# diffqc/dqc

Measured on AMD Instinct MI355X. Metric: SCF iterations/sec (Fock build + XC grid) per GPU, cc-pVDZ 20-atom, higher is better.
Workload: dtype f64

## Files before the change

dqc_amd/csrc/grid_density.hip:

```cpp
#include "grid_common.hpp"

namespace dqc {

constexpr int DEN_BM = 64;
constexpr int DEN_NT = DEN_BM * 4;
constexpr int DEN_KC = 16;
constexpr int DEN_SA = DEN_KC + 2;

#ifdef DEN_TRACE
__device__ long long g_den_trace[4 * 16384];
DQC_DEV void den_trace(int k) {
    if (threadIdx.x == 0 && blockIdx.x < 16384) {
        if (k == 0) {
            unsigned hw, xcc;
            asm volatile("s_getreg_b32 %0, hwreg(HW_REG_HW_ID)" : "=s"(hw));
            asm volatile("s_getreg_b32 %0, hwreg(HW_REG_XCC_ID)" : "=s"(xcc));
            g_den_trace[4 * blockIdx.x + 3] = (long long)(((xcc & 7u) << 8) | ((hw >> 8) & 0xffu));
        }
        g_den_trace[4 * blockIdx.x + k] = wall_clock64();
    }
}
#define DEN_TRACE_POINT(k) den_trace(k)
#else
#define DEN_TRACE_POINT(k)
#endif

#ifdef DEN_EXP_UNPAIRED
constexpr bool DEN_PAIRED = false;
#else
constexpr bool DEN_PAIRED = true;
#endif

constexpr int lr_panel_stride(int nct) {
    return (DEN_PAIRED && nct >= 2) ? nct * 16 + 1 : (((nct * 16) & 31) == 16 ? nct * 16 : nct * 16 + 16);
}

template <int NCT, bool GGA, int Q0 = 0>
DQC_DEV void rowdot_epilogue(const v4d (&acc)[NCT], double (&p)[4][GGA ? 4 : 1], const double *__restrict__ blk0,
                             const double *__restrict__ blkg, size_t cs, const int (&roff)[4], int col0) {
    constexpr int NQ = (GGA ? 4 : 1) - Q0, NB = 4 * NQ;
    if (NB == 0) return;
    constexpr int DP = 2;
    double t[DP][NCT];
    auto issue = [&](int bt, double (&dst)[NCT]) {
        const int r = bt / NQ, q = bt % NQ + Q0;
        const double *base = (q == 0 ? blk0 : blkg + q * cs) + col0;
#pragma unroll
        for (int ct = 0; ct < NCT; ct++) dst[ct] = base[roff[r] + ct * 16];
    };
#pragma unroll
    for (int b0 = 0; b0 < DP - 1 && b0 < NB; b0++) issue(b0, t[b0]);
#pragma unroll
    for (int bt = 0; bt < NB; bt++) {
        if (bt + DP - 1 < NB) issue(bt + DP - 1, t[(bt + DP - 1) % DP]);
        const int r = bt / NQ, q = bt % NQ + Q0;
#pragma unroll
        for (int ct = 0; ct < NCT; ct++) p[r][q] += acc[ct][r] * t[bt % DP][ct];
        __builtin_amdgcn_sched_barrier(0);
    }
}

template <int NCT, bool GGA, int Q0 = 0>
DQC_DEV void rowdot_epilogue_paired(const v4d (&acc)[NCT], double (&p)[4][GGA ? 4 : 1], const double *__restrict__ blk0,
                                    const double *__restrict__ blkg, size_t cs, const int (&roff)[4], int lr, int col0) {
    constexpr int NQ = (GGA ? 4 : 1) - Q0, NB = 4 * NQ, NP = NCT / 2, ODD = NCT & 1, DP = 2;
    if (NB == 0) return;
    double2 t2[DP][NP > 0 ? NP : 1];
    double t1[DP];
    auto issue = [&](int bt, double2 (&d2)[NP > 0 ? NP : 1], double &d1) {
        const int r = bt / NQ, q = bt % NQ + Q0;
        const double *base = (q == 0 ? blk0 : blkg + q * cs) + col0;
#pragma unroll
        for (int m = 0; m < NP; m++) d2[m] = *reinterpret_cast<const double2 *>(base + roff[r] + m * 32);
        if (ODD) d1 = base[(roff[r] - lr) + (NCT - 1) * 16];
    };
    issue(0, t2[0], t1[0]);
#pragma unroll
    for (int bt = 0; bt < NB; bt++) {
        if (bt + 1 < NB) issue(bt + 1, t2[(bt + 1) % DP], t1[(bt + 1) % DP]);
        const int r = bt / NQ, q = bt % NQ + Q0;
#pragma unroll
        for (int m = 0; m < NP; m++) p[r][q] += acc[2 * m][r] * t2[bt % DP][m].x + acc[2 * m + 1][r] * t2[bt % DP][m].y;
        if (ODD) p[r][q] += acc[NCT - 1][r] * t1[bt % DP];
        __builtin_amdgcn_sched_barrier(0);
    }
}

template <int NCT>
DQC_DEV void rowdot_epilogue_paired2(const v4d (&acc)[2][NCT], double (&p)[2][4][4], const double *__restrict__ blkg, size_t cs,
                                     const int (&roff)[4], int lr, int col0) {
    constexpr int NQ = 3, NB = 4 * NQ, NP = NCT / 2, ODD = NCT & 1, DP = 2;
    double2 t2[DP][NP > 0 ? NP : 1];
    double t1[DP];
    auto issue = [&](int bt, double2 (&d2)[NP > 0 ? NP : 1], double &d1) {
        const int r = bt / NQ, q = bt % NQ + 1;
        const double *base = blkg + q * cs + col0;
#pragma unroll
        for (int m = 0; m < NP; m++) d2[m] = *reinterpret_cast<const double2 *>(base + roff[r] + m * 32);
        if (ODD) d1 = base[(roff[r] - lr) + (NCT - 1) * 16];
    };
    issue(0, t2[0], t1[0]);
#pragma unroll
    for (int bt = 0; bt < NB; bt++) {
        if (bt + 1 < NB) issue(bt + 1, t2[(bt + 1) % DP], t1[(bt + 1) % DP]);
        const int r = bt / NQ, q = bt % NQ + 1;
#pragma unroll
        for (int sp = 0; sp < 2; sp++) {
#pragma unroll
            for (int m = 0; m < NP; m++) p[sp][r][q] += acc[sp][2 * m][r] * t2[bt % DP][m].x + acc[sp][2 * m + 1][r] * t2[bt % DP][m].y;
            if (ODD) p[sp][r][q] += acc[sp][NCT - 1][r] * t1[bt % DP];
        }
        __builtin_amdgcn_sched_barrier(0);
    }
}

template <int NCT, bool GGA>
__global__ __launch_bounds__(256, 2) void density_kernel(double *__restrict__ rho, double *__restrict__ grho,
                                                         const double *__restrict__ ao, int ngrid, int ld,
                                                         const double *__restrict__ dm, int ntile,
                                                         const double *__restrict__ aoe, int lda) {
    extern __shared__ __attribute__((aligned(16))) double lds[];
    constexpr int LSB = NCT * 16;
    constexpr int LSBP = lr_panel_stride(NCT);
    constexpr int A_SZ = DEN_BM * DEN_SA, B_SZ = DEN_KC * LSBP;
    constexpr int NB2 = (DEN_KC * LSB / 2 + DEN_NT - 1) / DEN_NT;
    constexpr int NKK = DEN_KC / 4;
    double *sA = lds, *sB = lds + 2 * A_SZ;
    const int tid = threadIdx.x, wave = tid >> 6, lane = tid & 63;
    const int lr = lane & 15, lk = lane >> 4;
    const int g0 = blockIdx.x * DEN_BM;
    const size_t cs = (size_t)ngrid * lda;
    const double *aoblk = ao + (size_t)g0 * lda;
    const double *aoeblk = aoe + (size_t)g0 * lda;
    const int rmax = ngrid - 1 - g0;
    const int arow = tid >> 2, aseg = (tid & 3) * 4;
    const int aoff = min(arow, rmax) * lda + aseg;

    double p[4][GGA ? 4 : 1];
#pragma unroll
    for (int r = 0; r < 4; r++)
#pragma unroll
        for (int q = 0; q < (GGA ? 4 : 1); q++) p[r][q] = 0.0;
    int roff[4];
#pragma unroll
    for (int r = 0; r < 4; r++) roff[r] = min(wave * 16 + lk + 4 * r, rmax) * lda + (DEN_PAIRED ? 2 : 1) * lr;

    DEN_TRACE_POINT(0);
    const int nk = ld / DEN_KC;
    for (int jnew = 0; jnew < ntile; jnew += NCT) {
        const int jc = min(jnew, ntile - NCT);
        v4d acc[NCT];
#pragma unroll
        for (int ct = 0; ct < NCT; ct++) acc[ct] = v4d{0, 0, 0, 0};
        double2 paA0 = make_double2(0.0, 0.0), paA1 = paA0, paB0 = paA0, paB1 = paA0, pbA[NB2], pbB[NB2];
        int boff[NB2];
        bool bzero[NB2];
#pragma unroll
        for (int i = 0; i < NB2; i++) {
            const int e = min((tid + i * DEN_NT) * 2, DEN_KC * LSB - 2);
            const int row = e / LSB, col = e - row * LSB;
            boff[i] = row * ld + jc * 16 + col;
            bzero[i] = jc * 16 + col < jnew * 16;
            pbA[i] = pbB[i] = make_double2(0.0, 0.0);
        }
#define DQC_DEN_PREF(KC, S, PART)                                                                          \
    {                                                                                                      \
        const int kq_ = min((KC), nk - 1);      \
        if ((PART) == 0) {                                                                                 \
            const double *s_ = aoblk + kq_ * DEN_KC + aoff;                                                \
            pa##S##0 = *reinterpret_cast<const double2 *>(s_);                                             \
            pa##S##1 = *reinterpret_cast<const double2 *>(s_ + 2);                                         \
        }                                                                                                  \
        const double *d_ = dm + (size_t)kq_ * DEN_KC * ld;                                                 \
        _Pragma("unroll") for (int i = 0; i < NB2; i++) {                                                  \
            if (i % NKK != (PART)) continue;                                                               \
            pb##S[i] = *reinterpret_cast<const double2 *>(d_ + boff[i]);                                   \
            if (bzero[i]) pb##S[i] = make_double2(0.0, 0.0);                                               \
        }                                                                                                  \
    }
#define DQC_DEN_STAGE(KC, S)                                                                               \
    if ((KC) < nk) {                                                                                       \
        const int buf_ = (KC) & 1;                                                                         \
        double *a_ = sA + buf_ * A_SZ + arow * DEN_SA + aseg;                                              \
        *reinterpret_cast<double2 *>(a_) = pa##S##0;                                                       \
        *reinterpret_cast<double2 *>(a_ + 2) = pa##S##1;                                                   \
        _Pragma("unroll") for (int i = 0; i < NB2; i++) {                                                  \
            const int e = (tid + i * DEN_NT) * 2;                                                          \
            const int row = e / LSB, col = e - row * LSB;                                                  \
            if (row < DEN_KC) {                                     \
                double *d = sB + buf_ * B_SZ + row * LSBP + col;                                           \
                d[0] = pb##S[i].x;                                                                         \
                d[1] = pb##S[i].y;                                                                         \
            }                                                                                              \
        }                                                                                                  \
    }
#define DQC_DEN_MFMAS(KC, S)                                                                               \
    {                                                                                                      \
        const int buf_ = (KC) & 1;                                                                         \
        const double *a = sA + buf_ * A_SZ + (wave * 16 + lr) * DEN_SA + lk;                               \
        const double *b = sB + buf_ * B_SZ + lk * LSBP + lr;                                               \
        const double *b2 = b + lr;  \
        _Pragma("unroll") for (int kk = 0; kk < NKK; kk++) {                                               \
            DQC_DEN_PREF((KC) + 2, S, kk)                     \
            const double av = a[kk * 4];                                                                   \
            _Pragma("unroll") for (int ct = 0; ct < NCT; ct++) {                                           \
                const double bv = (DEN_PAIRED && ct < 2 * (NCT / 2)) ? b2[kk * 4 * LSBP + 32 * (ct >> 1) + (ct & 1)] \
                                                                    : b[kk * 4 * LSBP + ct * 16];          \
                acc[ct] = mfma_f64(av, bv, acc[ct]);                                                       \
            }                                                                                              \
        }                                                                                                  \
    }
        __syncthreads();
#pragma unroll
        for (int part = 0; part < NKK; part++) DQC_DEN_PREF(0, A, part)
#pragma unroll
        for (int part = 0; part < NKK; part++) DQC_DEN_PREF(1, B, part)
        DQC_DEN_STAGE(0, A)
        __syncthreads();
        int kc = 0;
        for (; kc + 1 < nk; kc += 2) {
            DQC_DEN_MFMAS(kc, A)
            DQC_DEN_STAGE(kc + 1, B)
            __syncthreads();
            DQC_DEN_MFMAS(kc + 1, B)
            DQC_DEN_STAGE(kc + 2, A)
            __syncthreads();
        }
        if (kc < nk) {
            DQC_DEN_MFMAS(kc, A)
            __syncthreads();
        }
#undef DQC_DEN_PREF
// ... 187 lines not shown
        rs += __shfl_xor(rs, 32);
        const int row = g0 + wave * 16 + lr;
        if (lk == 0 && row < ngrid) rho[(size_t)sp * ngrid + row] = rs;
    }
    if (!GGA) return;

    double p[NS][4][GGA ? 4 : 1];
#pragma unroll
    for (int sp = 0; sp < NS; sp++)
#pragma unroll
    for (int r = 0; r < 4; r++)
#pragma unroll
        for (int q = 0; q < (GGA ? 4 : 1); q++) p[sp][r][q] = 0.0;
    int roff[4];
#pragma unroll
    for (int r = 0; r < 4; r++) roff[r] = min(wave * 16 + lk + 4 * r, rmax) * lda + (DEN_PAIRED ? 2 : 1) * lr;

    for (int jnew = 0; jnew < ntile; jnew += NCT) {
        const int jc = min(jnew, ntile - NCT);
        v4d acc[NS][NCT];
#pragma unroll
        for (int sp = 0; sp < NS; sp++)
#pragma unroll
        for (int ct = 0; ct < NCT; ct++) acc[sp][ct] = v4d{0, 0, 0, 0};
        double2 pb[NB2];
        int boff[NB2];
        bool bzero[NB2];
#pragma unroll
        for (int i = 0; i < NB2; i++) {
            const int e = min((tid + i * DEN_NT) * 2, DEN_KC * LSB - 2);
            const int row = e / LSB, col = e - row * LSB;
            boff[i] = row * ld + jc * 16 + col;
            bzero[i] = jc * 16 + col < jnew * 16;
        }
        auto prefetch = [&](int kc) {
            const double *l = orbt + (size_t)kc * DEN_KC * ld;
#pragma unroll
            for (int i = 0; i < NB2; i++) {
                pb[i] = *reinterpret_cast<const double2 *>(l + boff[i]);
                if (bzero[i]) pb[i] = make_double2(0.0, 0.0);
            }
        };
        auto stage = [&](int buf) {
#pragma unroll
            for (int i = 0; i < NB2; i++) {
                const int e = (tid + i * DEN_NT) * 2;
                const int row = e / LSB, col = e - row * LSB;
                if (row < DEN_KC) {
                    double *d = sB + buf * B_SZ + row * LSBP + col;
                    d[0] = pb[i].x;
                    d[1] = pb[i].y;
                }
            }
        };
        __syncthreads();
        prefetch(0);
        stage(0);
        __syncthreads();
#pragma unroll 1
        for (int kc = 0; kc < NRT; kc++) {
            const int buf = kc & 1;
            if (kc + 1 < NRT) prefetch(kc + 1);
            v4d a4 = a1[0];
#pragma unroll
            for (int c = 1; c < NRT; c++)
                if (kc == c) a4 = a1[c];
            const double *b = sB + buf * B_SZ + lk * LSBP + lr;
            const double *b2 = b + lr;
#pragma unroll
            for (int kk = 0; kk < 4; kk++) {
                const double av = a4[kk];
#pragma unroll
                for (int ct = 0; ct < NCT; ct++) {
                    const double bv = (DEN_PAIRED && ct < 2 * (NCT / 2)) ? b2[kk * 4 * LSBP + 32 * (ct >> 1) + (ct & 1)]
                                                                        : b[kk * 4 * LSBP + ct * 16];
                    if (NS == 1 || kc < NRU) acc[0][ct] = mfma_f64(av, bv, acc[0][ct]);
                    else acc[NS - 1][ct] = mfma_f64(av, bv, acc[NS - 1][ct]);
                }
            }
            if (kc + 1 < NRT) stage(buf ^ 1);
            __syncthreads();
        }
        DEN_TRACE_POINT(1);
        if constexpr (NS == 2) {
            static_assert(NS == 1 || (DEN_PAIRED && GGA), "spin-fused form: paired epilogue only");
            rowdot_epilogue_paired2<NCT>(acc, p, aoblk, cs, roff, lr, jc * 16);
        } else if constexpr (!DEN_PAIRED) rowdot_epilogue<NCT, GGA, 1>(acc[0], p[0], aoblk, aoblk, cs, roff, jc * 16);
        else if constexpr (GGA) rowdot_epilogue_paired<NCT, true, 1>(acc[0], p[0], aoblk, aoblk, cs, roff, lr, jc * 16);
        DEN_TRACE_POINT(2);
    }
#pragma unroll
    for (int sp = 0; sp < NS; sp++)
#pragma unroll
    for (int r = 0; r < 4; r++)
#pragma unroll
        for (int q = 0; q < (GGA ? 4 : 1); q++) {
            double v = p[sp][r][q];
            v += __shfl_xor(v, 1);
            v += __shfl_xor(v, 2);
            v += __shfl_xor(v, 4);
            v += __shfl_xor(v, 8);
            p[sp][r][q] = v;
        }
    if (lr == 0) {
#pragma unroll
        for (int sp = 0; sp < NS; sp++)
#pragma unroll
        for (int r = 0; r < 4; r++) {
            const int row = g0 + wave * 16 + lk + 4 * r;
            if (row < ngrid) {
                double *gs = grho + (size_t)sp * 3 * ngrid;
                gs[row] = 2.0 * p[sp][r][1];
                gs[(size_t)ngrid + row] = 2.0 * p[sp][r][2];
                gs[2 * (size_t)ngrid + row] = 2.0 * p[sp][r][3];
            }
        }
    }
}

template <int NRT, int NCT>
static constexpr size_t density_lr_lds_bytes() {
    constexpr int LSBP = lr_panel_stride(NCT);
    constexpr int RPS = LrGeom<NRT>::RPS;
    return sizeof(double) * 2 * (DEN_BM * DEN_SA + DEN_KC * (LSBP > RPS ? LSBP : RPS));
}

constexpr int lr_max_nct(int nrt) { return nrt <= 3 ? 14 : (nrt <= 4 ? 12 : 10); }

template <int NRT, bool GGA>
static int launch_density_lr_n(int nct, dim3 grid, hipStream_t st, double *rho, double *grho, const double *ao, int ngrid,
                               int ld, const double *orb, const double *orbt, int ntile, int lda) {
#define DQC_DLR_CASE(N)                                                                                          \
    case N:                                                                                                      \
        if constexpr (!GGA || N <= lr_max_nct(NRT)) {          \
            constexpr size_t shm = density_lr_lds_bytes<NRT, N>();                                               \
            auto kern = density_lr_kernel<NRT, N, GGA>;                                                          \
            (void)hipFuncSetAttribute((const void *)kern, hipFuncAttributeMaxDynamicSharedMemorySize, (int)shm); \
            hipLaunchKernelGGL(kern, grid, dim3(DEN_NT), shm, st, rho, grho, ao, ngrid, ld, orb, orbt, ntile, lda); \
            return 0;                                                                                            \
        }                                                                                                        \
        break;
    switch (nct) {
        DQC_DLR_CASE(1) DQC_DLR_CASE(2) DQC_DLR_CASE(3) DQC_DLR_CASE(4) DQC_DLR_CASE(5) DQC_DLR_CASE(6) DQC_DLR_CASE(7)
        DQC_DLR_CASE(8) DQC_DLR_CASE(9) DQC_DLR_CASE(10) DQC_DLR_CASE(11) DQC_DLR_CASE(12) DQC_DLR_CASE(13) DQC_DLR_CASE(14)
        DQC_DLR_CASE(15) DQC_DLR_CASE(16)
    default:
        break;
    }
#undef DQC_DLR_CASE
    set_error("density_lr: internal tile-count dispatch error");
    return DQC_EINVAL;
}

template <int NRT>
__global__ __launch_bounds__(256, 2) void density_lr_tau_kernel(double *__restrict__ rho, double *__restrict__ grho, double *__restrict__ tau,
                                                                const double *__restrict__ ao, int ngrid, int ld,
                                                                const double *__restrict__ orb, int lda) {
    extern __shared__ __attribute__((aligned(16))) double lds[];
    constexpr int RP = LrGeom<NRT>::RP, RPS = LrGeom<NRT>::RPS;
    constexpr int A_SZ = DEN_BM * DEN_SA, B_SZ = DEN_KC * RPS;
    constexpr int NL2 = (DEN_KC * RP / 2 + DEN_NT - 1) / DEN_NT;
    static_assert(NL2 <= 4, "L chunk wider than 4 double2 per thread");
    double *sA = lds, *sB = lds + 4 * A_SZ;
    const int tid = threadIdx.x, wave = tid >> 6, lane = tid & 63;
    const int lr = lane & 15, lk = lane >> 4;
    const int g0 = blockIdx.x * DEN_BM;
    const size_t cs = (size_t)ngrid * lda;
    const double *aoblk = ao + (size_t)g0 * lda;
    const int rmax = ngrid - 1 - g0;
    const int arow = tid >> 2, aseg = (tid & 3) * 4;
    const int aoff = min(arow, rmax) * lda + aseg;
    const int nk = ld / DEN_KC;
    const int lo0 = min((tid + 0 * DEN_NT) * 2, DEN_KC * RP - 2), lo1 = min((tid + 1 * DEN_NT) * 2, DEN_KC * RP - 2);
    const int lo2 = min((tid + 2 * DEN_NT) * 2, DEN_KC * RP - 2), lo3 = min((tid + 3 * DEN_NT) * 2, DEN_KC * RP - 2);

    v4d psi[NRT];
    double rs = 0.0, ts = 0.0, gs[3] = {0.0, 0.0, 0.0};
#pragma unroll 1
    for (int pair = 0; pair < 2; pair++) {
        const double *blk0 = aoblk + (size_t)(2 * pair) * cs, *blk1 = blk0 + cs;
        v4d a0[NRT], a1[NRT];
#pragma unroll
        for (int ct = 0; ct < NRT; ct++) a0[ct] = a1[ct] = v4d{0, 0, 0, 0};
        double2 x0a, x0b, y0a, y0b, x1a, x1b, y1a, y1b, pl0a, pl0b, pl0c, pl0d, pl1a, pl1b, pl1c, pl1d;
        pl0a = pl0b = pl0c = pl0d = pl1a = pl1b = pl1c = pl1d = make_double2(0.0, 0.0);
#define DQC_LT_PREFETCH(KC, S)                                                                            \
    {                                                                                                     \
        const int kq = min((KC), nk - 1);      \
        const double *s0_ = blk0 + kq * DEN_KC + aoff, *s1_ = blk1 + kq * DEN_KC + aoff;                  \
        x##S##a = *reinterpret_cast<const double2 *>(s0_);                                                \
        x##S##b = *reinterpret_cast<const double2 *>(s0_ + 2);                                            \
        y##S##a = *reinterpret_cast<const double2 *>(s1_);                                                \
        y##S##b = *reinterpret_cast<const double2 *>(s1_ + 2);                                            \
        const double *l_ = orb + (size_t)kq * DEN_KC * RP;                                                \
        pl##S##a = *reinterpret_cast<const double2 *>(l_ + lo0);                                          \
        if (NL2 > 1) pl##S##b = *reinterpret_cast<const double2 *>(l_ + lo1);                             \
        if (NL2 > 2) pl##S##c = *reinterpret_cast<const double2 *>(l_ + lo2);                             \
        if (NL2 > 3) pl##S##d = *reinterpret_cast<const double2 *>(l_ + lo3);                             \
    }
#define DQC_LT_PUT(I, V)                                                                                  \
    {                                                                                                     \
        const int e_ = (tid + (I) * DEN_NT) * 2;                                                          \
        const int row_ = e_ / RP, col_ = e_ - row_ * RP;                                                  \
        if (row_ < DEN_KC) *reinterpret_cast<double2 *>(sB + buf_ * B_SZ + row_ * RPS + col_) = V;        \
    }
#define DQC_LT_STAGE(KC, S)                                                                               \
    if ((KC) < nk) {                                                                                      \
        const int buf_ = (KC) & 1;                                                                        \
        double *a_ = sA + buf_ * 2 * A_SZ + arow * DEN_SA + aseg;                                         \
        *reinterpret_cast<double2 *>(a_) = x##S##a;                                                       \
        *reinterpret_cast<double2 *>(a_ + 2) = x##S##b;                                                   \
        *reinterpret_cast<double2 *>(a_ + A_SZ) = y##S##a;                                                \
        *reinterpret_cast<double2 *>(a_ + A_SZ + 2) = y##S##b;                                            \
        DQC_LT_PUT(0, pl##S##a)                                                                           \
        if (NL2 > 1) DQC_LT_PUT(1, pl##S##b)                                                              \
        if (NL2 > 2) DQC_LT_PUT(2, pl##S##c)                                                              \
        if (NL2 > 3) DQC_LT_PUT(3, pl##S##d)                                                              \
    }
#define DQC_LT_MFMAS(KC)                                                                                  \
    {                                                                                                     \
        const int buf_ = (KC) & 1;                                                                        \
        const double *b_ = sA + buf_ * 2 * A_SZ + (wave * 16 + lr) * DEN_SA + lk;  \
        const double *l_ = sB + buf_ * B_SZ + lk * RPS + lr;                       \
        _Pragma("unroll") for (int kk = 0; kk < DEN_KC / 4; kk++) {                                       \
            const double bv0 = b_[kk * 4], bv1 = b_[A_SZ + kk * 4];                                       \
            _Pragma("unroll") for (int ct = 0; ct < NRT; ct++) {                                          \
                const double lv = l_[kk * 4 * RPS + ct * 16];                                             \
                a0[ct] = mfma_f64(lv, bv0, a0[ct]);                                                       \
                a1[ct] = mfma_f64(lv, bv1, a1[ct]);                                                       \
            }                                                                                             \
        }                                                                                                 \
    }
        __syncthreads();
        DQC_LT_PREFETCH(0, 0)
        DQC_LT_PREFETCH(1, 1)
        DQC_LT_STAGE(0, 0)
        __syncthreads();
        int kc = 0;
        for (; kc + 1 < nk; kc += 2) {
            DQC_LT_PREFETCH(kc + 2, 0)
            DQC_LT_MFMAS(kc)
            DQC_LT_STAGE(kc + 1, 1)
            __syncthreads();
            DQC_LT_PREFETCH(kc + 3, 1)
            DQC_LT_MFMAS(kc + 1)
            DQC_LT_STAGE(kc + 2, 0)
            __syncthreads();
        }
        if (kc < nk) {
            DQC_LT_MFMAS(kc)
            __syncthreads();
        }
#undef DQC_LT_PREFETCH
#undef DQC_LT_STAGE
#undef DQC_LT_PUT
#undef DQC_LT_MFMAS
        if (pair == 0) {
#pragma unroll
            for (int ct = 0; ct < NRT; ct++) {
                psi[ct] = a0[ct];
#pragma unroll
                for (int q = 0; q < 4; q++) {
                    rs += a0[ct][q] * a0[ct][q];
                    gs[0] += a0[ct][q] * a1[ct][q];
                    ts += a1[ct][q] * a1[ct][q];
                }
            }
        } else {
#pragma unroll
            for (int ct = 0; ct < NRT; ct++)
#pragma unroll
                for (int q = 0; q < 4; q++) {
                    gs[1] += psi[ct][q] * a0[ct][q];
                    gs[2] += psi[ct][q] * a1[ct][q];
                    ts += a0[ct][q] * a0[ct][q] + a1[ct][q] * a1[ct][q];
                }
        }
    }
    double out[5] = {rs, 2.0 * gs[0], 2.0 * gs[1], 2.0 * gs[2], 0.5 * ts};
#pragma unroll
    for (int q = 0; q < 5; q++) {
        out[q] += __shfl_xor(out[q], 16);
        out[q] += __shfl_xor(out[q], 32);
    }
    const int row = g0 + wave * 16 + lr;
    if (lk == 0 && row < ngrid) {
        rho[row] = out[0];
        grho[row] = out[1];
        grho[(size_t)ngrid + row] = out[2];
        grho[2 * (size_t)ngrid + row] = out[3];
        tau[row] = out[4];
    }
}

constexpr int lr2_max_nct(int nrt) { return nrt <= 4 ? 6 : (nrt <= 6 ? 5 : 4); }

template <int NRT>
static int launch_density_lr2_n(int nct, dim3 grid, hipStream_t st, double *rho, double *grho, const double *ao, int ngrid, int ld,
                                const double *orb, const double *orbt, int ntile, int lda) {
#define DQC_DLR2_CASE(N)                                                                                         \
    case N:                                                                                                      \
        if constexpr (N <= lr2_max_nct(NRT)) {                                                                   \
            constexpr size_t shm = density_lr_lds_bytes<NRT, N>();                                               \
            auto kern = density_lr_kernel<NRT, N, true, 2>;                                                      \
            (void)hipFuncSetAttribute((const void *)kern, hipFuncAttributeMaxDynamicSharedMemorySize, (int)shm); \
            hipLaunchKernelGGL(kern, grid, dim3(DEN_NT), shm, st, rho, grho, ao, ngrid, ld, orb, orbt, ntile, lda); \
            return 0;                                                                                            \
        }                                                                                                        \
        break;
    switch (nct) {
        DQC_DLR2_CASE(1) DQC_DLR2_CASE(2) DQC_DLR2_CASE(3) DQC_DLR2_CASE(4) DQC_DLR2_CASE(5) DQC_DLR2_CASE(6) DQC_DLR2_CASE(7)
    default:
        break;
    }
#undef DQC_DLR2_CASE
    set_error("density_lr (two spins): internal tile-count dispatch error");
    return DQC_EINVAL;
}

template <bool GGA>
static int launch_density_lr(int nrt, int nct, dim3 grid, hipStream_t st, double *rho, double *grho, const double *ao,
                             int ngrid, int ld, const double *orb, const double *orbt, int ntile, int lda) {
    switch (nrt) {
    case 1: return launch_density_lr_n<1, GGA>(nct, grid, st, rho, grho, ao, ngrid, ld, orb, orbt, ntile, lda);
    case 2: return launch_density_lr_n<2, GGA>(nct, grid, st, rho, grho, ao, ngrid, ld, orb, orbt, ntile, lda);
    case 3: return launch_density_lr_n<3, GGA>(nct, grid, st, rho, grho, ao, ngrid, ld, orb, orbt, ntile, lda);
    case 4: return launch_density_lr_n<4, GGA>(nct, grid, st, rho, grho, ao, ngrid, ld, orb, orbt, ntile, lda);
    case 6: return launch_density_lr_n<6, GGA>(nct, grid, st, rho, grho, ao, ngrid, ld, orb, orbt, ntile, lda);
    case 8: return launch_density_lr_n<8, GGA>(nct, grid, st, rho, grho, ao, ngrid, ld, orb, orbt, ntile, lda);
    default:
        set_error("density_lr: internal factor-width dispatch error");
        return DQC_EINVAL;
    }
}

}

extern "C" {

int dqc_grid_density(double *d_rho, double *d_grho, const double *d_ao, int ncomp, int ngrid, int nao,
                     const double *d_dm, void *stream) {
    using namespace dqc;
    hipStream_t st = (hipStream_t)stream;
    if (ngrid <= 0) return DQC_OK;
    const bool gga = d_grho != nullptr;
    if (gga && ncomp < 4) { set_error("dqc_grid_density: gradient requested but ao has < 4 components"); return DQC_EINVAL; }
    const int ld = dqc_padded_nao(nao), ntile = ld / 16, lda = dqc_ao_stride(nao);
    const int nchunk = (ntile + (gga ? 13 : 15)) / (gga ? 14 : 16);
    const int nct = (ntile + nchunk - 1) / nchunk;
    dim3 grid((ngrid + DEN_BM - 1) / DEN_BM);
    int rc = gga ? launch_density<true>(nct, grid, st, d_rho, d_grho, d_ao, ngrid, ld, d_dm, ntile, d_ao, lda)
                 : launch_density<false>(nct, grid, st, d_rho, d_grho, d_ao, ngrid, ld, d_dm, ntile, d_ao, lda);
    if (rc) return rc;
    DQC_CHECK_LAUNCH();
    return DQC_OK;
}

int dqc_padded_norb(int norb) {
    static const int sizes[] = {16, 32, 48, 64, 96, 128};
    for (int sz : sizes)
        if (norb <= sz) return sz;
    return 0;
}

int dqc_grid_density_lr(double *d_rho, double *d_grho, const double *d_ao, int ncomp, int ngrid, int nao,
                        const double *d_orb, const double *d_orbt, int norb_pad, void *stream) {
    using namespace dqc;
    hipStream_t st = (hipStream_t)stream;
    if (ngrid <= 0) return DQC_OK;
    const bool gga = d_grho != nullptr;
    if (gga && ncomp < 4) { set_error("dqc_grid_density_lr: gradient requested but ao has < 4 components"); return DQC_EINVAL; }
    if (norb_pad <= 0 || dqc_padded_norb(norb_pad) != norb_pad) {
        set_error("dqc_grid_density_lr: norb_pad must be a value returned by dqc_padded_norb");
        return DQC_EINVAL;
    }
    const int ld = dqc_padded_nao(nao), ntile = ld / 16, lda = dqc_ao_stride(nao);
    const int lim = gga ? dqc::lr_max_nct(norb_pad / 16) : 16;
    const int nchunk = (ntile + lim - 1) / lim;
    const int nct = (ntile + nchunk - 1) / nchunk;
    dim3 grid((ngrid + DEN_BM - 1) / DEN_BM);
    int rc = gga ? launch_density_lr<true>(norb_pad / 16, nct, grid, st, d_rho, d_grho, d_ao, ngrid, ld, d_orb, d_orbt, ntile, lda)
                 : launch_density_lr<false>(norb_pad / 16, nct, grid, st, d_rho, d_grho, d_ao, ngrid, ld, d_orb, d_orbt, ntile, lda);
    if (rc) return rc;
    DQC_CHECK_LAUNCH();
    return DQC_OK;
}

int dqc_grid_density_lr_pol(double *d_rho, double *d_grho, const double *d_ao, int ncomp, int ngrid, int nao,
                            const double *d_orb, const double *d_orbt, int norb_pad_spin, void *stream) {
    using namespace dqc;
    hipStream_t st = (hipStream_t)stream;
    if (ngrid <= 0) return DQC_OK;
    if (!d_grho || ncomp < 4) { set_error("dqc_grid_density_lr_pol: needs the four AO components and the gradient output"); return DQC_EINVAL; }
    if (norb_pad_spin != 16 && norb_pad_spin != 32 && norb_pad_spin != 48 && norb_pad_spin != 64) {
        set_error("dqc_grid_density_lr_pol: norb_pad_spin must be 16, 32, 48 or 64");
        return DQC_EINVAL;
    }
    const int ld = dqc_padded_nao(nao), ntile = ld / 16, lda = dqc_ao_stride(nao);
    const int nrt = 2 * norb_pad_spin / 16;
    const int lim = lr2_max_nct(nrt);
    const int nchunk = (ntile + lim - 1) / lim;
    const int nct = (ntile + nchunk - 1) / nchunk;
    dim3 grid((ngrid + DEN_BM - 1) / DEN_BM);
    int rc;
    switch (nrt) {
    case 2: rc = launch_density_lr2_n<2>(nct, grid, st, d_rho, d_grho, d_ao, ngrid, ld, d_orb, d_orbt, ntile, lda); break;
    case 4: rc = launch_density_lr2_n<4>(nct, grid, st, d_rho, d_grho, d_ao, ngrid, ld, d_orb, d_orbt, ntile, lda); break;
    case 6: rc = launch_density_lr2_n<6>(nct, grid, st, d_rho, d_grho, d_ao, ngrid, ld, d_orb, d_orbt, ntile, lda); break;
    default: rc = launch_density_lr2_n<8>(nct, grid, st, d_rho, d_grho, d_ao, ngrid, ld, d_orb, d_orbt, ntile, lda); break;
    }
    if (rc) return rc;
    DQC_CHECK_LAUNCH();
    return DQC_OK;
}

int dqc_grid_density_pair(double *d_out, const double *d_ao_a, const double *d_ao_b, int ngrid, int nao,
                          const double *d_dm, void *stream) {
    using namespace dqc;
    hipStream_t st = (hipStream_t)stream;
    if (ngrid <= 0) return DQC_OK;
    const int ld = dqc_padded_nao(nao), ntile = ld / 16, lda = dqc_ao_stride(nao);
    const int nchunk = (ntile + 15) / 16;
    const int nct = (ntile + nchunk - 1) / nchunk;
    dim3 grid((ngrid + DEN_BM - 1) / DEN_BM);
    int rc = launch_density<false>(nct, grid, st, d_out, nullptr, d_ao_a, ngrid, ld, d_dm, ntile, d_ao_b, lda);
    if (rc) return rc;
    DQC_CHECK_LAUNCH();
    return DQC_OK;
}

int dqc_grid_density_lr_tau(double *d_rho, double *d_grho, double *d_tau, const double *d_ao, int ncomp, int ngrid, int nao,
                            const double *d_orb, int norb_pad, void *stream) {
    using namespace dqc;
    hipStream_t st = (hipStream_t)stream;
    if (ngrid <= 0) return DQC_OK;
    if (ncomp < 4 || !d_grho || !d_tau) { set_error("dqc_grid_density_lr_tau: needs the four AO components and all three outputs"); return DQC_EINVAL; }
    if (norb_pad <= 0 || dqc_padded_norb(norb_pad) != norb_pad) {
        set_error("dqc_grid_density_lr_tau: norb_pad must be a value returned by dqc_padded_norb");
        return DQC_EINVAL;
    }
    const int ld = dqc_padded_nao(nao), lda = dqc_ao_stride(nao);
    dim3 grid((ngrid + DEN_BM - 1) / DEN_BM);
#define DQC_LT_CASE(N)                                                                                                         \
    case N: {                                                                                                                  \
        constexpr size_t bytes = sizeof(double) * (4 * DEN_BM * DEN_SA + 2 * DEN_KC * LrGeom<N>::RPS);                         \
        (void)hipFuncSetAttribute((const void *)density_lr_tau_kernel<N>, hipFuncAttributeMaxDynamicSharedMemorySize, (int)bytes); \
        hipLaunchKernelGGL((density_lr_tau_kernel<N>), grid, dim3(DEN_NT), bytes, st, d_rho, d_grho, d_tau, d_ao, ngrid, ld, d_orb, lda); \
    } break;
    switch (norb_pad / 16) {
        DQC_LT_CASE(1) DQC_LT_CASE(2) DQC_LT_CASE(3) DQC_LT_CASE(4) DQC_LT_CASE(6)
    default:
        set_error("dqc_grid_density_lr_tau: factors wider than 96 columns are not supported");
        return DQC_EINVAL;
    }
#undef DQC_LT_CASE
    DQC_CHECK_LAUNCH();
    return DQC_OK;
}

}
```

include/dqc_amd.h:

```cpp
#ifndef DQC_AMD_H
#define DQC_AMD_H
#include <stddef.h>
#include <stdint.h>

#ifdef __cplusplus
extern "C" {
#endif

#define DQC_OK 0
#define DQC_EINVAL (-1)
#define DQC_EHIP (-2)
#define DQC_ENOMEM (-3)

const char *dqc_last_error(void);
int dqc_version(void);
int dqc_nao(const int *bas, int nbas);
int dqc_padded_nao(int nao);
int dqc_ao_stride(int nao);
size_t dqc_ao_doubles(int ncomp, int ngrid, int nao);

int dqc_int1e(int which, double *d_out, const int *atm, int natm, const int *bas, int nbas,
              const double *env, int nenv, const double *zs, void *stream);

size_t dqc_eri_tile_count(int nao);
size_t dqc_eri_store_doubles(int nao);
int dqc_eri_fill_tiles(double *d_tiles, const int *atm, int natm, const int *bas, int nbas,
                       const double *env, int nenv, void *stream);
int dqc_eri_pair_stats(const int *atm, int natm, const int *bas, int nbas, const double *env, int nenv, int merge, long long *h_out);

int dqc_eri_tiles_to_dense(double *d_dense, const double *d_tiles, int nao, void *stream);

size_t dqc_jk_work_doubles(int nao);
int dqc_jk_from_tiles(double *d_J, double *d_K, const double *d_tiles, const double *d_dm,
                      int nao, double *d_work, void *stream);

int dqc_fock_max_nao(void);
int dqc_fock_factor(double *d_orb, double *d_orbt, const double *d_x, const double *d_c, int ldc, const double *d_w, int nao, int north,
                    int r, int ld, int rp, void *stream);
int dqc_fock_orb2dm(double *d_dm, double *d_orb, double *d_orbt, const double *d_x, const double *d_c, int ldc, const double *d_w, int nao,
                    int north, int r, int ld, int rp, void *stream);
int dqc_fock_prep(double *d_work, const double *d_dm, const double *d_x, const double *d_orb, int rp, int nao, int north, int with_k,
                  void *stream);
int dqc_jk_stream_prepared(const double *d_tiles, int nao, double *d_work, int with_k, void *stream);
int dqc_fock_finish_vraw(double *d_fock, double *d_energies, double *d_work, const double *d_vxc_raw, int ldv, double vscale,
                         const double *d_core, const double *d_x, int nao, int north, void *stream);
int dqc_fock_finish(double *d_fock, double *d_energies, double *d_j_ao, double *d_work, const double *d_vxc_ao, int ldv,
                    const double *d_core, const double *d_x, int nao, int north, int with_k, void *stream);

size_t dqc_jk_multi_work_doubles(int nao, int nj, int nk);
int dqc_jk_from_tiles_multi(double *d_J, const double *d_dmJ, int nj, double *d_K, const double *d_dmK, int nk,
                            const double *d_tiles, int nao, double *d_work, void *stream);

int dqc_eval_gto(int deriv, double *d_out, const double *d_coords, int ngrid, const int *atm,
                 int natm, const int *bas, int nbas, const double *env, int nenv, void *stream);

int dqc_grid_density(double *d_rho, double *d_grho, const double *d_ao, int ncomp, int ngrid,
                     int nao, const double *d_dm, void *stream);


#define DQC_XC_LDA_X 1
#define DQC_XC_LDA_C_VWN 7
#define DQC_XC_LDA_C_PZ 9
#define DQC_XC_LDA_C_PW 12
#define DQC_XC_LDA_C_PW_MOD 13
#define DQC_XC_GGA_X_PBE 101
#define DQC_XC_GGA_X_PBE_R 102
#define DQC_XC_GGA_X_B86 103
#define DQC_XC_GGA_X_B88 106
#define DQC_XC_GGA_X_G96 107
#define DQC_XC_GGA_X_PW86 108
#define DQC_XC_GGA_X_PW91 109
#define DQC_XC_GGA_X_OPTX 110
#define DQC_XC_GGA_X_WC 118
#define DQC_XC_GGA_X_PBE_SOL 116
#define DQC_XC_GGA_X_RPBE 117
#define DQC_XC_GGA_C_PBE 130
#define DQC_XC_GGA_C_LYP 131
#define DQC_XC_GGA_C_P86 132
#define DQC_XC_GGA_C_PBE_SOL 133
#define DQC_XC_MGGA_X_TPSS 202
#define DQC_XC_MGGA_C_TPSS 231
#define DQC_XC_MGGA_X_SCAN 263
#define DQC_XC_MGGA_C_SCAN 267
int dqc_xc_eval(double *d_edens, double *d_vrho, double *d_vgrad, const double *d_rho,
                const double *d_grho, int n, const int *ids, const double *coefs, int nterm,
                void *stream);

#define DQC_XC_QUAD_DOUBLES 1025
int dqc_xc_eval_quad(double *d_exc, double *d_edens, double *d_vrho, double *d_vgrad, const double *d_rho,
                     const double *d_grho, const double *d_w, int n, const int *ids, const double *coefs, int nterm,
                     void *stream);
int dqc_xc_eval_pol(double *d_edens, double *d_vrho_u, double *d_vrho_d, double *d_vgrad_u, double *d_vgrad_d,
                    const double *d_rho_u, const double *d_rho_d, const double *d_grho_u, const double *d_grho_d,
                    int n, const int *ids, const double *coefs, int nterm, void *stream);

int dqc_xc_eval_mgga(double *d_edens, double *d_vrho, double *d_vgrad, double *d_vtau, const double *d_rho,
                     const double *d_grho, const double *d_tau, int n, const int *ids, const double *coefs,
                     int nterm, void *stream);

int dqc_xc_eval_mgga_pol(double *d_edens, double *d_vrho_u, double *d_vrho_d, double *d_vgrad, double *d_vtau,
                         const double *d_rho_u, const double *d_rho_d, const double *d_grho_u, const double *d_grho_d,
                         const double *d_tau_u, const double *d_tau_d, int n, const int *ids, const double *coefs, int nterm,
                         void *stream);

int dqc_xc_eval_mgga_pol2(double *d_edens, double *d_vrho_u, double *d_vrho_d, double *d_vgrad_u, double *d_vgrad_d,
                          double *d_vtau, const double *d_rho_u, const double *d_rho_d, const double *d_grho_u,
                          const double *d_grho_d, const double *d_tau_u, const double *d_tau_d, int n, const int *ids,
                          const double *coefs, int nterm, void *stream);

int dqc_int3c2e(double *d_j3c, const int *atm, int natm, const int *bas, int nbas, const double *env, int nenv,
                int sh0, int sh1, int k0, int k1, void *stream);
int dqc_int2c2e(double *d_j2c, const int *atm, int natm, const int *bas, int nbas, const double *env, int nenv,
                int k0, int k1, void *stream);

int dqc_df_coulomb(double *d_j, const double *d_j3c, const double *d_inv_j2c, const double *d_dm_ao, int nao,
                   int naux, double *d_work, void *stream);

int dqc_ncart(const int *bas, int nbas);
int dqc_cart2sph_matrix(double *h_out, const int *bas, int nbas);
int dqc_int1e_grad(double *d_grad, const double *d_dcart, const double *d_wcart, const int *atm, int natm,
                   const int *bas, int nbas, const double *env, int nenv, const double *zs, void *stream);
int dqc_eri_grad(double *d_grad, const double *d_dcart, double jscale, double kscale, const int *atm, int natm, const int *bas,
                 int nbas, const double *env, int nenv, void *stream);
int dqc_int1e_potential(double *d_out, const double *d_dcart, const double *d_points, int npts, const int *atm, int natm,
                        const int *bas, int nbas, const double *env, int nenv, void *stream);
int dqc_df_grad(double *d_grad, const double *d_dcart, const double *d_ccart, const int *atm, int natm, const int *bas,
                int nbas, const double *env, int nenv, int sh0, int sh1, int k0, int k1, void *stream);

int dqc_becke_weights(double *d_w, const double *d_xyz, const int *d_atom_off, const double *d_pos,
                      const double *d_inv_rij, const double *d_aij, int natm, int ngrid, double cut, void *stream);
int dqc_becke_weights_grad(double *d_gpos, double *d_gxyz, double *d_scratch, const double *d_cw, const double *d_xyz,
                           const int *d_atom_off, const double *d_pos, const double *d_inv_rij, const double *d_aij,
                           int natm, int ngrid, double cut, void *stream);

int dqc_purify_tc2(double *d_x, double *d_tmp, int ld, double nocc, int iters, double tol, double *d_state,
                   void *stream);
int dqc_purify_tc2_persist(double *d_x, double *d_tmp, int ld, double nocc, int iters, double tol, double *d_state,
                           unsigned *d_ctl, void *stream);
size_t dqc_projector_work_doubles(int n, int iters);
int dqc_projector_tc2(double *d_p, double *d_err, const double *d_fock, int n, double nocc, int iters, double tol, double *d_work,
                      void *stream);

int dqc_orth_factor(double *d_q, const double *d_y, const double *d_g, int n, int r, void *stream);

int dqc_purify_tc2_batched(double *d_x, double *d_tmp, int ld, int nmol, double nocc, int iters, double tol,
                           double *d_state, void *stream);
int dqc_orth_factor_batched(double *d_q, const double *d_y, const double *d_g, int n, int r, int nmol, void *stream);
int dqc_diis_solve(double *d_c, const double *d_gram, int nmol, int nhist, int m, void *stream);
int dqc_diis_solve_dev(double *d_c, const double *d_gram, int nmol, int nhist, const long long *d_count, void *stream);

int dqc_grid_vxc(double *d_vmat, const double *d_ao, int ncomp, int ngrid, int nao,
                 const double *d_w, const double *d_vrho, const double *d_vgrad, void *stream);

int dqc_padded_norb(int norb);
int dqc_grid_density_lr(double *d_rho, double *d_grho, const double *d_ao, int ncomp, int ngrid, int nao,
                        const double *d_orb, const double *d_orbt, int norb_pad, void *stream);
int dqc_grid_density_lr_pol(double *d_rho, double *d_grho, const double *d_ao, int ncomp, int ngrid, int nao,
                            const double *d_orb, const double *d_orbt, int norb_pad_spin, void *stream);

int dqc_grid_xc_gradient_terms(double *d_q, double *d_perao, const double *d_ao, int ngrid, int nao, const double *d_b,
                               const double *d_c0, const double *d_c1, const double *d_c2, int ldb, const double *d_w,
                               const double *d_vrho, const double *d_u, const double *d_grho, const double *d_vtau, void *stream);

int dqc_grid_density_lr_tau(double *d_rho, double *d_grho, double *d_tau, const double *d_ao, int ncomp, int ngrid, int nao,
                            const double *d_orb, int norb_pad, void *stream);

int dqc_grid_density_pair(double *d_out, const double *d_ao_a, const double *d_ao_b, int ngrid, int nao,
                          const double *d_dm, void *stream);
int dqc_grid_vxc_pair(double *d_vmat, const double *d_ao_a, const double *d_ao_b, int ngrid, int nao,
                      const double *d_w, const double *d_v, void *stream);

int dqc_grid_vxc_raw(double *d_vmat, const double *d_ao, int ncomp, int ngrid, int nao, const double *d_w, const double *d_vrho,
                     const double *d_vgrad, double *h_scale, void *stream);

long long dqc_eri_tile_offset(int nao, long long tile);
int dqc_eri_fill_tiles_part(double *d_tiles_part, const int *atm, int natm, const int *bas, int nbas, const double *env, int nenv,
                            long long tile_begin, long long tile_end, void *stream);
int dqc_jk_from_tiles_part(double *d_J, double *d_K, const double *d_tiles_part, const double *d_dm, int nao, double *d_work,
                           long long tile_begin, long long tile_end, void *stream);

int dqc_jk_direct(double *d_J, double *d_K, const double *d_dm, const int *atm, int natm, const int *bas, int nbas,
                  const double *env, int nenv, void *stream);

int dqc_direct_create(void **ctx, const int *atm, int natm, const int *bas, int nbas, const double *env, int nenv, void *stream);
int dqc_direct_jk(void *ctx, double *d_J, double *d_K, const double *d_dm, double tau, void *stream);
int dqc_direct_jk_part(void *ctx, double *d_J, double *d_K, const double *d_dm, double tau, int part, int nparts, void *stream);
int dqc_direct_stats(void *ctx, long long *quartets_total, long long *quartets_launched, double *dmax);
int dqc_direct_npairs(void *ctx);
int dqc_direct_bounds(void *ctx, double *h_q, int *h_shells);
int dqc_direct_bounds_groups(void *ctx, double *h_q, int *h_shells, int *h_group);
int dqc_direct_destroy(void *ctx);

int dqc_set_deterministic(int on);
int dqc_get_deterministic(void);

int dqc_set_generic_eri(int on);

int dqc_device_cu_count(void);
int dqc_stream_create_partition(void **stream_out, int cu_begin, int cu_end, int priority);
int dqc_stream_destroy(void *stream);
int dqc_stream_cus(void *stream);
int dqc_set_vxc_cus(int ncu);

int dqc_probe_stream_read(const double *d_buf, size_t n, double *d_out, void *stream);
int dqc_probe_mfma_f64(double *d_out, int iters, void *stream);

#ifdef __cplusplus
}
#endif
#endif
```

Before: 765.4.

## Add warp-specialized persistent density kernel with producer/consumer waves for GGA shape

Adds a persistent kernel for one specific shape (3 orbital tiles, 13 AO tiles). Four producer waves compute the orbital products with MFMA and hand them through LDS mailboxes to four consumer waves that run the gradient row-dot epilogue, with flag-based handoff between the two groups. The whole orbital matrix stays resident in LDS, and the epilogue prefetch depth becomes a template parameter set to 3 here. It aims to overlap the GEMM and epilogue phases and cut redundant global loads, at the cost of one block per CU, spin-wait synchronization, and a NaN fallback if a wait times out.

Result: faster. 794.1, median of 6 (+3.8%).

```diff
diff --git a/dqc_amd/csrc/grid_density.hip b/dqc_amd/csrc/grid_density.hip
--- a/dqc_amd/csrc/grid_density.hip
+++ b/dqc_amd/csrc/grid_density.hip
@@ -60,10 +60,10 @@
     }
 }
 
-template <int NCT, bool GGA, int Q0 = 0>
+template <int NCT, bool GGA, int Q0 = 0, int DP = 2>
 DQC_DEV void rowdot_epilogue_paired(const v4d (&acc)[NCT], double (&p)[4][GGA ? 4 : 1], const double *__restrict__ blk0,
                                     const double *__restrict__ blkg, size_t cs, const int (&roff)[4], int lr, int col0) {
-    constexpr int NQ = (GGA ? 4 : 1) - Q0, NB = 4 * NQ, NP = NCT / 2, ODD = NCT & 1, DP = 2;
+    constexpr int NQ = (GGA ? 4 : 1) - Q0, NB = 4 * NQ, NP = NCT / 2, ODD = NCT & 1;
     if (NB == 0) return;
     double2 t2[DP][NP > 0 ? NP : 1];
     double t1[DP];
@@ -74,10 +74,11 @@
         for (int m = 0; m < NP; m++) d2[m] = *reinterpret_cast<const double2 *>(base + roff[r] + m * 32);
         if (ODD) d1 = base[(roff[r] - lr) + (NCT - 1) * 16];
     };
-    issue(0, t2[0], t1[0]);
+#pragma unroll
+    for (int b0 = 0; b0 < DP - 1 && b0 < NB; b0++) issue(b0, t2[b0], t1[b0]);
 #pragma unroll
     for (int bt = 0; bt < NB; bt++) {
-        if (bt + 1 < NB) issue(bt + 1, t2[(bt + 1) % DP], t1[(bt + 1) % DP]);
+        if (bt + DP - 1 < NB) issue(bt + DP - 1, t2[(bt + DP - 1) % DP], t1[(bt + DP - 1) % DP]);
         const int r = bt / NQ, q = bt % NQ + Q0;
 #pragma unroll
         for (int m = 0; m < NP; m++) p[r][q] += acc[2 * m][r] * t2[bt % DP][m].x + acc[2 * m + 1][r] * t2[bt % DP][m].y;
@@ -571,6 +572,242 @@
     return DQC_EINVAL;
 }
 
+constexpr int ROLE_NT = 512;
+constexpr unsigned ROLE_SPIN_CAP = 1u << 22;
+constexpr int ROLE_DP = 3;
+
+template <int NRT, int NT>
+struct RoleGeom {
+    static constexpr int RP = NRT * 16;
+    static constexpr int S = NT * 16 + 1;
+    static constexpr int P0 = (NT + 1) / 2;
+    static constexpr int P1 = NT - P0;
+    static constexpr int LT_SZ = (RP * S + 1) & ~1;
+    static constexpr int MB_W = P0 * 256;
+    static constexpr int SA_W = 2 * 16 * DEN_SA;
+    static constexpr size_t lds_bytes() { return sizeof(double) * (LT_SZ + 4 * MB_W + 4 * SA_W) + 64; }
+};
+
+template <int NT>
+DQC_DEV int role_col(int ct, int lr) {
+    return ct < 2 * (NT / 2) ? 32 * (ct >> 1) + 2 * lr + (ct & 1) : ct * 16 + lr;
+}
+
+DQC_DEV void role_wait(unsigned *flag, unsigned want, unsigned *broken) {
+    unsigned n = 0;
+    while (__hip_atomic_load(flag, __ATOMIC_ACQUIRE, __HIP_MEMORY_SCOPE_WORKGROUP) < want) {
+        if (__hip_atomic_load(broken, __ATOMIC_RELAXED, __HIP_MEMORY_SCOPE_WORKGROUP) != 0u) break;
+        if (++n > ROLE_SPIN_CAP) {
+            __hip_atomic_store(broken, 1u, __ATOMIC_RELAXED, __HIP_MEMORY_SCOPE_WORKGROUP);
+            break;
+        }
+        __builtin_amdgcn_s_sleep(2);
+    }
+}
+
+DQC_DEV void role_signal(unsigned *flag, unsigned v) {
+    __hip_atomic_store(flag, v, __ATOMIC_RELEASE, __HIP_MEMORY_SCOPE_WORKGROUP);
+}
+
+template <int NRT, int NT>
+__global__ __launch_bounds__(ROLE_NT, 1) void density_roles_kernel(double *__restrict__ rho, double *__restrict__ grho,
+                                                                   const double *__restrict__ ao, int ngrid,
+                                                                   const double *__restrict__ orbt, int lda) {
+    using G = RoleGeom<NRT, NT>;
+    constexpr int RP = G::RP, S = G::S, P0 = G::P0, P1 = G::P1, LD = NT * 16;
+    constexpr int NPF = 4;
+    static_assert(NT >= 2 && NT <= 14 && P1 >= 1, "one epilogue panel of 2..14 tiles");
+    extern __shared__ __attribute__((aligned(16))) double lds[];
+    double *sLT = lds, *sMB = lds + G::LT_SZ, *sAall = sMB + 4 * G::MB_W;
+    unsigned *flags = reinterpret_cast<unsigned *>(sAall + 4 * G::SA_W);
+    const int tid = threadIdx.x, lane = tid & 63;
+    const int wave = __builtin_amdgcn_readfirstlane(tid >> 6);
+    const int lr = lane & 15, lk = lane >> 4;
+    const int ntiles = (ngrid + DEN_BM - 1) / DEN_BM;
+    const size_t cs = (size_t)ngrid * lda;
+
+    for (int e = tid; e < RP * LD; e += ROLE_NT) {
+        const int r = e / LD, c = e - r * LD;
+        sLT[r * S + c] = orbt[e];
+    }
+    if (tid < 16) flags[tid] = 0u;
+    __syncthreads();
+    const int w = wave & 3;
+    unsigned *filled = flags + w, *drained = flags + 4 + w, *broken = flags + 8;
+    double *mb = sMB + w * G::MB_W + lane * 2;
+    unsigned seq = 0;
+
+    if (wave < 4) {
+        double *sA = sAall + w * G::SA_W;
+        const int arow = lane >> 2, aseg = (lane & 3) * 4;
+        double2 pa0a, pa0b, pa1a, pa1b, pa2a, pa2b, pa3a, pa3b;
+        static_assert(NPF == 4, "four named prefetch sets");
+#define DQC_ROLE_REQUEST(T, KC, SET)                                                                       \
+    {                                                         \
+        const int rmax_ = ngrid - 1 - (T) * DEN_BM;                                                        \
+        const double *s_ = ao + (size_t)(T) * DEN_BM * lda + (min(w * 16 + arow, rmax_) * lda + aseg) + (KC) * DEN_KC; \
+        pa##SET##a = *reinterpret_cast<const double2 *>(s_);                                               \
+        pa##SET##b = *reinterpret_cast<const double2 *>(s_ + 2);                                           \
+    }
+#define DQC_ROLE_STEP(KC, SET)                                                                             \
+    if ((KC) < NT) {                                                                                       \
+        double *a_ = sA + ((KC) & 1) * 16 * DEN_SA;                                                        \
+        *reinterpret_cast<double2 *>(a_ + arow * DEN_SA + aseg) = pa##SET##a;                              \
+        *reinterpret_cast<double2 *>(a_ + arow * DEN_SA + aseg + 2) = pa##SET##b;                          \
+        if ((KC) + NPF < NT) DQC_ROLE_REQUEST(t, (KC) + NPF, SET)                                          \
+        __builtin_amdgcn_fence(__ATOMIC_RELEASE, "wavefront");                                             \
+        __builtin_amdgcn_wave_barrier();  \
+        __builtin_amdgcn_fence(__ATOMIC_ACQUIRE, "wavefront");                                             \
+        const double *b_ = a_ + lr * DEN_SA + lk;                            \
+        const double *l_ = sLT + lr * S + (KC) * DEN_KC + lk;                \
+        _Pragma("unroll") for (int kk = 0; kk < DEN_KC / 4; kk++) {                                        \
+            const double bv = b_[kk * 4];                                                                  \
+            _Pragma("unroll") for (int ct = 0; ct < NRT; ct++)                                             \
+                a1[ct] = mfma_f64(l_[ct * 16 * S + kk * 4], bv, a1[ct]);                                   \
+        }                                                                                                  \
+    }
+#define DQC_ROLE_REQUEST4(T)  \
+    DQC_ROLE_REQUEST(T, 0, 0) DQC_ROLE_REQUEST(T, 1, 1) DQC_ROLE_REQUEST(T, 2, 2) DQC_ROLE_REQUEST(T, 3, 3)
+        int t = blockIdx.x;
+        pa0a = pa0b = pa1a = pa1b = pa2a = pa2b = pa3a = pa3b = make_double2(0.0, 0.0);
+        if (t < ntiles) { DQC_ROLE_REQUEST4(t) }
+        for (; t < ntiles; t += gridDim.x) {
+            const int g0 = t * DEN_BM;
+            v4d a1[NRT];
+#pragma unroll
+            for (int ct = 0; ct < NRT; ct++) a1[ct] = v4d{0, 0, 0, 0};
+            DQC_ROLE_STEP(0, 0) DQC_ROLE_STEP(1, 1) DQC_ROLE_STEP(2, 2) DQC_ROLE_STEP(3, 3) DQC_ROLE_STEP(4, 0)
+            DQC_ROLE_STEP(5, 1) DQC_ROLE_STEP(6, 2) DQC_ROLE_STEP(7, 3) DQC_ROLE_STEP(8, 0) DQC_ROLE_STEP(9, 1)
+            DQC_ROLE_STEP(10, 2) DQC_ROLE_STEP(11, 3) DQC_ROLE_STEP(12, 0) DQC_ROLE_STEP(13, 1)
+            {
+                double rs = 0.0;
+#pragma unroll
+                for (int ct = 0; ct < NRT; ct++)
+#pragma unroll
+                    for (int q = 0; q < 4; q++) rs += a1[ct][q] * a1[ct][q];
+                rs += __shfl_xor(rs, 16);
+                rs += __shfl_xor(rs, 32);
+                const int row = g0 + w * 16 + lr;
+                if (lk == 0 && row < ngrid) rho[row] = rs;
+            }
+            if (t + (int)gridDim.x < ntiles) { DQC_ROLE_REQUEST4(t + (int)gridDim.x) }
+#pragma unroll
+            for (int h = 0; h < 2; h++) {
+                constexpr int PMAX = P0;
+                const int c0 = h * P0;
+                v4d acc[PMAX];
+#pragma unroll
+                for (int ct = 0; ct < PMAX; ct++) acc[ct] = v4d{0, 0, 0, 0};
+#pragma unroll
+                for (int kc = 0; kc < NRT; kc++)
+#pragma unroll
+                    for (int kk = 0; kk < 4; kk++) {
+                        const double av = a1[kc][kk];
+                        const double *b = sLT + (kc * 16 + kk * 4 + lk) * S;
+#pragma unroll
+                        for (int ct = 0; ct < PMAX; ct++)
+                            if (ct < (h ? P1 : P0)) acc[ct] = mfma_f64(av, b[role_col<NT>(c0 + ct, lr)], acc[ct]);
+                    }
+                role_wait(drained, seq, broken);
+#pragma unroll
+                for (int ct = 0; ct < PMAX; ct++)
+                    if (ct < (h ? P1 : P0)) {
+                        *reinterpret_cast<double2 *>(mb + (2 * ct) * 128) = make_double2(acc[ct][0], acc[ct][1]);
+                        *reinterpret_cast<double2 *>(mb + (2 * ct + 1) * 128) = make_double2(acc[ct][2], acc[ct][3]);
+                    }
+                seq++;
+                role_signal(filled, seq);
+            }
+        }
+#undef DQC_ROLE_REQUEST4
+#undef DQC_ROLE_STEP
+#undef DQC_ROLE_REQUEST
+    } else {
+        for (int t = blockIdx.x; t < ntiles; t += gridDim.x) {
+            const int g0 = t * DEN_BM;
+            const int rmax = ngrid - 1 - g0;
+            const double *aoblk = ao + (size_t)g0 * lda;
+            int roff[4];
+#pragma unroll
+            for (int r = 0; r < 4; r++) roff[r] = min(w * 16 + lk + 4 * r, rmax) * lda + 2 * lr;
+            v4d acc[NT];
+#pragma unroll
+            for (int h = 0; h < 2; h++) {
+                role_wait(filled, seq + 1, broken);
+#pragma unroll
+                for (int ct = 0; ct < (h ? P1 : P0); ct++) {
+                    const double2 lo = *reinterpret_cast<const double2 *>(mb + (2 * ct) * 128);
+                    const double2 hi = *reinterpret_cast<const double2 *>(mb + (2 * ct + 1) * 128);
+                    acc[h * P0 + ct] = v4d{lo.x, lo.y, hi.x, hi.y};
+                }
+                seq++;
+                role_signal(drained, seq);
+            }
+            double p[4][4];
+#pragma unroll
+            for (int r = 0; r < 4; r++)
+#pragma unroll
+                for (int q = 0; q < 4; q++) p[r][q] = 0.0;
+            rowdot_epilogue_paired<NT, true, 1, ROLE_DP>(acc, p, aoblk, aoblk, cs, roff, lr, 0);
+#pragma unroll
+            for (int r = 0; r < 4; r++)
+#pragma unroll
+                for (int q = 1; q < 4; q++) {
+                    double v = p[r][q];
+                    v += __shfl_xor(v, 1);
+                    v += __shfl_xor(v, 2);
+                    v += __shfl_xor(v, 4);
+                    v += __shfl_xor(v, 8);
+                    p[r][q] = v;
+                }
+            const bool bad = __hip_atomic_load(broken, __ATOMIC_RELAXED, __HIP_MEMORY_SCOPE_WORKGROUP) != 0u;
+            if (lr == 0) {
+#pragma unroll
+                for (int r = 0; r < 4; r++) {
+                    const int row = g0 + w * 16 + lk + 4 * r;
+                    if (row < ngrid) {
+                        const double nan = __builtin_nan("");
+                        grho[row] = bad ? nan : 2.0 * p[r][1];
+                        grho[(size_t)ngrid + row] = bad ? nan : 2.0 * p[r][2];
+                        grho[2 * (size_t)ngrid + row] = bad ? nan : 2.0 * p[r][3];
+                    }
+                }
+            }
+        }
+    }
+}
+
+static bool density_roles_shape(int nrt, int ntile) { return nrt == 3 && ntile == 13; }
+
+static bool density_roles_enabled() {
+    const char *e = getenv("DQC_DENSITY_ROLES");
+    return !(e && e[0] == '0');
+}
+
+static int launch_density_roles(int nrt, int ntile, hipStream_t st, double *rho, double *grho, const double *ao, int ngrid,
+                                const double *orbt, int lda) {
+    static int ncu = 0;
+    if (ncu == 0) {
+        int dev = 0, n = 0;
+        if (hipGetDevice(&dev) != hipSuccess || hipDeviceGetAttribute(&n, hipDeviceAttributeMultiprocessorCount, dev) != hipSuccess || n <= 0) {
+            set_error("density_roles: cannot read the device's CU count");
+            return DQC_EINVAL;
+        }
+        ncu = n;
+    }
+    const int ntiles = (ngrid + DEN_BM - 1) / DEN_BM;
+    if (nrt == 3 && ntile == 13) {
+        constexpr size_t shm = RoleGeom<3, 13>::lds_bytes();
+        static_assert(shm <= 160 * 1024, "one block has to fit the CU's LDS");
+        auto kern = density_roles_kernel<3, 13>;
+        (void)hipFuncSetAttribute((const void *)kern, hipFuncAttributeMaxDynamicSharedMemorySize, (int)shm);
+        hipLaunchKernelGGL(kern, dim3(std::min(ntiles, ncu)), dim3(ROLE_NT), shm, st, rho, grho, ao, ngrid, orbt, lda);
+        return 0;
+    }
+    set_error("density_roles: internal shape dispatch error");
+    return DQC_EINVAL;
+}
+
 template <int NRT>
 __global__ __launch_bounds__(256, 2) void density_lr_tau_kernel(double *__restrict__ rho, double *__restrict__ grho, double *__restrict__ tau,
                                                                 const double *__restrict__ ao, int ngrid, int ld,
@@ -798,11 +1035,21 @@
     const int nchunk = (ntile + lim - 1) / lim;
     const int nct = (ntile + nchunk - 1) / nchunk;
     dim3 grid((ngrid + DEN_BM - 1) / DEN_BM);
-    int rc = gga ? launch_density_lr<true>(norb_pad / 16, nct, grid, st, d_rho, d_grho, d_ao, ngrid, ld, d_orb, d_orbt, ntile, lda)
+    int rc;
+    if (gga && density_roles_shape(norb_pad / 16, ntile) && density_roles_enabled())
+        rc = launch_density_roles(norb_pad / 16, ntile, st, d_rho, d_grho, d_ao, ngrid, d_orbt, lda);
+    else
+        rc = gga ? launch_density_lr<true>(norb_pad / 16, nct, grid, st, d_rho, d_grho, d_ao, ngrid, ld, d_orb, d_orbt, ntile, lda)
                  : launch_density_lr<false>(norb_pad / 16, nct, grid, st, d_rho, d_grho, d_ao, ngrid, ld, d_orb, d_orbt, ntile, lda);
     if (rc) return rc;
     DQC_CHECK_LAUNCH();
     return DQC_OK;
+}
+
+int dqc_grid_density_lr_roles(int nao, int norb_pad, int gga) {
+    using namespace dqc;
+    if (!gga || norb_pad <= 0 || dqc_padded_norb(norb_pad) != norb_pad) return 0;
+    return density_roles_shape(norb_pad / 16, dqc_padded_nao(nao) / 16) && density_roles_enabled() ? 1 : 0;
 }
 
 int dqc_grid_density_lr_pol(double *d_rho, double *d_grho, const double *d_ao, int ncomp, int ngrid, int nao,
diff --git a/include/dqc_amd.h b/include/dqc_amd.h
--- a/include/dqc_amd.h
+++ b/include/dqc_amd.h
@@ -155,6 +155,7 @@
 int dqc_padded_norb(int norb);
 int dqc_grid_density_lr(double *d_rho, double *d_grho, const double *d_ao, int ncomp, int ngrid, int nao,
                         const double *d_orb, const double *d_orbt, int norb_pad, void *stream);
+int dqc_grid_density_lr_roles(int nao, int norb_pad, int gga);
 int dqc_grid_density_lr_pol(double *d_rho, double *d_grho, const double *d_ao, int ncomp, int ngrid, int nao,
                             const double *d_orb, const double *d_orbt, int norb_pad_spin, void *stream);
 
```
